# imazen/image-webp

Hardware: AMD Instinct MI355X
Metric: 1920x1080 lossy encodes/s (Q75, method 4) (higher is better)
Workload: dtype int32; 1 GPU; encode_frame_lossy 1920x1080 RGBA Q75 m4; device_batch=1024, distinct_frames=4, mbs_per_frame=8160, parallelism=frames sharded over 1 GPU(s), steps_pipelined=True, pipeline_lanes=2

## Files before the change

image-webp_amd/csrc/zw_enc_kernels.hip:

```cpp
#include "zw_dev.h"

#include <type_traits>

#include "zw_enc_rows.h"
#include "zw_enc_pairfinal.h"

#define ZW_PH_N 28

#ifdef ZW_NW
#define ZW_NW1 ZW_NW
#define ZW_NW2 ZW_NW
#endif
#ifndef ZW_NW1
#define ZW_NW1 12
#endif
#ifndef ZW_NW2
#define ZW_NW2 12
#endif
#define NW_MAX (ZW_NW1 > ZW_NW2 ? ZW_NW1 : ZW_NW2)
#ifndef ZW_DYN_PRIO
#define ZW_DYN_PRIO 1
#endif
#ifndef ZW_DYN_PRIO1
#define ZW_DYN_PRIO1 2
#endif
#ifndef ZW_P1_LUMA_MAX
#define ZW_P1_LUMA_MAX 3
#endif
#ifndef ZW_CHAIN_PRIO
#define ZW_CHAIN_PRIO 3
#endif
#ifndef ZW_LUMA_PRIO
#define ZW_LUMA_PRIO 0
#endif

template <int PASS> struct PassShape {
    static constexpr int NW = PASS == 1 ? ZW_NW1 : ZW_NW2;
    static constexpr int WG = NW * 64;
};

struct EncArgs {
    const uint8_t *Y, *U, *V;
    const uint8_t* alpha;
    const ZwFrameParams* params;
    const ZwLevelCosts* lcost;
    int8_t* derr;
    ZwMbOut* out;
    uint8_t *ry, *ru, *rv;
    size_t ysz, csz;
    int mbw, mbh, pass;
    int* dbg;
    uint8_t* rows;
    uint32_t* sizes;
    int nframes;
};

struct MbLds {
    uint8_t sy[256], su[64], sv[64];
    uint8_t ws[17 * ZW_BPS];
    uint8_t left_y[20], left_u[12], left_v[12], left_c[12];
    int8_t left_derr[4];
    uint8_t modes[16];
    int16_t lev[25][16];
};

struct WaveLds {
    MbLds mb;
    uint8_t cu[9 * ZW_BPS], cv[9 * ZW_BPS];
    uint32_t uvc[64][8];
    int dc[64];
    int y2d[64];
    int y2cost[4];
    int V[2][40];
    int nzt[4], nzl[4];
    int misc[16];
    uint32_t pst[2][4];
    uint8_t win_y[32], win_u[8], win_v[8], win_c[12];
    int8_t win_d[4];
#ifdef ZW_PHASE_PROF
    unsigned long long ph[ZW_PH_N];
#endif
};


struct Ctx {
    const EncArgs* a;
    const ZwFrameParams* P;
    int method;
    const ZwSegment* S;
    const ZwSegment* Sl;
    const LdsTables* T;
    WaveLds* W;
    MbLds* M;
    uint8_t *top_y, *top_u, *top_v, *top_c;
    int8_t* top_derr;
    const uint8_t *srcY, *srcU, *srcV;
    const uint8_t *sY, *sU, *sV;
    int ys, cs;
    int mbx, mby, lane, seg;
    int f;
    int oy, oc, ocx, od;
};

__device__ void build_luma_border(const Ctx& C, int part = 2)
{
    uint8_t* ws = C.M->ws;
    const int l = C.lane;
    const int mbw = C.a->mbw;
    const bool want = part == 2 || (part == 0 ? (l < 17 || l >= 32) : (l >= 17 && l < 32));
    if (!want) {
    } else if (l < 32) {
        int v;
        if (l == 0) v = C.mby == 0 ? 127 : (C.mbx == 0 ? 129 : C.M->left_y[0]);
        else if (C.mby == 0) v = 127;
        else if (l <= 16) v = C.top_y[C.oy + l - 1];
        else if (C.mbx == mbw - 1) v = C.top_y[C.oy + 15];
        else v = C.top_y[C.oy + l - 1];
        ws[l] = (uint8_t)v;
        if (l >= 17 && l < 21) {
            ws[4 * ZW_BPS + l] = (uint8_t)v;
            ws[8 * ZW_BPS + l] = (uint8_t)v;
            ws[12 * ZW_BPS + l] = (uint8_t)v;
        }
    } else if (l < 48) {
        int i = l - 32;
        ws[(i + 1) * ZW_BPS] = C.mbx == 0 ? 129 : C.M->left_y[1 + i];
    }
    wsync();
}

__device__ void build_chroma_border(const Ctx& C)
{
    const int l = C.lane;
    if (l < 34) {
        const int pl = l >= 17;
        const int i = pl ? l - 17 : l;
        uint8_t* w = pl ? C.W->cv : C.W->cu;
        const uint8_t* top = pl ? C.top_v : C.top_u;
        const uint8_t* left = pl ? C.M->left_v : C.M->left_u;
        if (i == 0) w[0] = C.mby == 0 ? 127 : (C.mbx == 0 ? 129 : left[0]);
        else if (i <= 8) w[i] = C.mby == 0 ? 127 : top[C.oc + i - 1];
        else w[(i - 8) * ZW_BPS] = C.mbx == 0 ? 129 : left[i - 8];
    }
    wsync();
}

template <int PASS>
__device__ void pick_i16(const Ctx& C, int& best_mode, unsigned long long& best_score)
{
    const int lane = C.lane, m = lane >> 4, b = lane & 15, bx = b & 3, by = b >> 2;
    const uint8_t* ws = C.M->ws;
    const ZwSegment& S = *C.S;
    const LdsTables* T = C.T;
    const int above = C.mby != 0, left = C.mbx != 0;
    int dcv;
    {
        const int top = lane < 16;
        const int v = (int)ws[csel(top, 1 + b, (b + 1) * ZW_BPS)] & -(int)(lane < 32 && (top ? above : left));
        const int sum = red16(v);
        const int s = __builtin_amdgcn_readlane(sum, 0) + __builtin_amdgcn_readlane(sum, 16);
        const int shf = 3 + above + left;
        dcv = (!above && !left) ? 128 : ((s + (1 << (shf - 1))) >> shf);
    }
    int src[16], pr[16], r[16], c[16];
    {
        const int P0 = ws[0];
        int L[4], Tp[4];
#pragma unroll
        for (int i = 0; i < 4; i++) {
            L[i] = ws[(by * 4 + i + 1) * ZW_BPS];
            Tp[i] = ws[1 + bx * 4 + i];
        }
#pragma unroll
        for (int i = 0; i < 4; i++) {
            const uint32_t srow = *(const uint32_t*)(C.sY + (by * 4 + i) * 16 + bx * 4);
#pragma unroll
            for (int j = 0; j < 4; j++) {
                const int p = sel4(m, dcv, Tp[j], L[i], clamp255(L[i] + Tp[j] - P0));
                const int sv = (int)((srow >> (8 * j)) & 255u);
                src[i * 4 + j] = sv;
                pr[i * 4 + j] = p;
                r[i * 4 + j] = sv - p;
            }
        }
    }
    fdct16_pk(r, c);
    int aq[16], dq[16];
    aq[0] = 0;
    int nzac = 0;
#pragma unroll
    for (int k = 1; k < 16; k++) {
        aq[k] = (int)((__umul24((uint32_t)iabs(c[k]), S.y1.iq[1]) + S.y1.bias[1]) >> 17);
        nzac |= aq[k];
        dq[k] = m24(c[k] < 0 ? -aq[k] : aq[k], (int)S.y1.q[1]);
    }
    nzac = nzac != 0;
    int cost = (int)rcost_bf<1, PASS == 2>(aq, 0, 0, T);
    int y2cost;
    {
        const int d = wht_g(c[0], b);
        const int t = b > 0;
        const int ay = (int)((__umul24((uint32_t)iabs(d), S.y2.iq[t]) + S.y2.bias[t]) >> 17);
        const int qy = d < 0 ? -ay : ay;
        y2cost = (int)rcost_g<0, PASS == 2>(qy, b, 0, 1, T);
        dq[0] = iwht_g(m24(qy, (int)S.y2.q[t]), b);
    }
    idct16(dq);
    int rec[16], sse = 0, flat = 1;
    const int s00 = C.sY[0];
#pragma unroll
    for (int k = 0; k < 16; k++) {
        rec[k] = clamp255(pr[k] + dq[k]);
        const int d = src[k] - rec[k];
        sse += m24(d, d);
        flat &= src[k] == s00;
    }
    int td = iabs(ttransform_diff_pk(rec, src)) >> 5;
    sse = red16(sse);
    td = red16(td);
    cost = red16(cost);
    nzac = red16(nzac);
    flat = red16(flat);
    const int srcflat = __builtin_amdgcn_readlane(flat, 0) == 16;
    cost += y2cost;
    int sd = S.tlambda > 0 ? ((int)S.tlambda * td + 128) >> 8 : 0;
    int dfin = sse;
    if (srcflat && nzac == 0) {
        dfin = sse * 2;
        sd = sd * 2;
    }
    const int mcost = sel4(m, d_FIXED_COSTS_I16[0], d_FIXED_COSTS_I16[1], d_FIXED_COSTS_I16[2], d_FIXED_COSTS_I16[3]) + cost;
    const int dist = dfin + sd;
    long long brd = 0x7fffffffffffffffLL, bfin = 0;
    int bm = 0;
#pragma unroll
    for (int mm = 0; mm < 4; mm++) {
        const long long mc = __builtin_amdgcn_readlane(mcost, mm * 16);
        const long long dd = 256LL * __builtin_amdgcn_readlane(dist, mm * 16);
        const long long r_m = mc * (long long)S.l_i16 + dd;
        const long long f_m = mc * (long long)S.l_mode + dd;
        const int avail = mm == 0 || (mm == 1 && above) || (mm == 2 && left) || (mm == 3 && above && left);
        if (avail && r_m < brd) {
            brd = r_m;
            bfin = f_m;
            bm = mm;
        }
    }
    best_mode = bm;
    best_score = bfin < 0 ? 0ull : (unsigned long long)bfin;
}

#ifdef ZW_PHASE_PROF
__device__ unsigned long long zw_phase_cycles_dev[2][ZW_PH_N];
__device__ unsigned long long zw_wave_cycles_dev[2][16][ZW_PH_N];
#define PH_START() long long ph_t_ = clock64()
#define PH_RESET() (ph_t_ = clock64())
#define PH_MARK(k) PH_MARK_L(k, lane, PASS)
#define PH_MARK_L(k, ln, ps)                                                        \
    do {                                                                            \
        const long long n_ = clock64();                                             \
        if ((ln) == 0) C.W->ph[k] += (unsigned long long)(n_ - ph_t_);               \
        ph_t_ = n_;                                                                 \
    } while (0)
extern "C" int zw_wave_cycles(unsigned long long* out, int reset)
{
    if (hipMemcpyFromSymbol(out, HIP_SYMBOL(zw_wave_cycles_dev), sizeof(zw_wave_cycles_dev)) != hipSuccess) return -1;
    if (reset) {
        static unsigned long long z[2][16][ZW_PH_N];
        if (hipMemcpyToSymbol(HIP_SYMBOL(zw_wave_cycles_dev), z, sizeof z) != hipSuccess) return -1;
    }
    return 0;
}
extern "C" int zw_phase_cycles(unsigned long long* out, int reset)
{
    if (hipMemcpyFromSymbol(out, HIP_SYMBOL(zw_phase_cycles_dev), sizeof(zw_phase_cycles_dev)) != hipSuccess) return -1;
    if (reset) {
        static unsigned long long z[2][ZW_PH_N];
        if (hipMemcpyToSymbol(HIP_SYMBOL(zw_phase_cycles_dev), z, sizeof z) != hipSuccess) return -1;
    }
    return 0;
}
#define PH_COUNT(k) \
    do {                \
        if (C.lane == 0) C.W->ph[k] += 1; \
    } while (0)
#else
#define PH_COUNT(k) (void)0
#define PH_START() (void)0
#define PH_RESET() (void)0
#define PH_MARK(k) (void)0
#define PH_MARK_L(k, ln, ps) (void)0
#endif

template <int NB>
__device__ __forceinline__ void i4_values_n(const Ctx& C, const int* x0, const int* y0)
{
    WaveLds* W = C.W;
    const uint8_t* ws = C.M->ws;
    const int l = C.lane;
    const int t = (int)(l >= 13) + (int)(l >= 24) + (int)(l >= 36) + (int)(l >= 37);
    const int k = min(l - 13 * (int)(l >= 13) - 11 * (int)(l >= 24), 12);
    const int t3 = (int)(t == 3), t4 = (int)(t >= 4), t12 = (int)(t == 1 || t == 2);
    const int ka = k + t3 * (11 - k) + t4 * (1 - k);
    const int kb = k + t12 + t3 * (12 - k) - t4 * k;
    const int kc = min(k + 2 * (int)(t == 1), 12);
    const int wb = 2 * (int)(t == 1) + (int)(t == 2) + 3 * (t3 + t4);
    const int wc = (int)(t == 1);
    const int sh = (int)(t != 0) + (int)(t != 0 && t != 2);
// ... 490 lines not shown
    const uint32_t rate = (uint32_t)(mcost + cost);
    const uint32_t score = (uint32_t)sse * 256u + (rate & 0xffffu) * S.l_i4;
    const uint32_t key2 = k < K ? (score << 2) | (uint32_t)k : 0xffffffffu;
    const uint32_t kmin = min16u(key2);
    const unsigned long long win = __ballot(key2 == kmin);
    PH_MARK_L(12, l, 0);
    int bk[NB];
#pragma unroll
    for (int h = 0; h < NB; h++) {
        bk[h] = __builtin_ctz((uint32_t)(win >> (16 * h)) & 0xffffu) >> 2;
        const int bmode = (int)((modes >> (16 * h + 4 * bk[h])) & 15u);
        const int wl = 16 * h + 4 * bk[h];
        const uint32_t bsse = (uint32_t)__builtin_amdgcn_readlane(sse, wl);
        const uint32_t brate = (uint32_t)__builtin_amdgcn_readlane((int)rate, wl);
        const int bnz = __builtin_amdgcn_readlane((int)(last >= 0), wl);
        const int i = sby[h] * 4 + sbx[h];
        st.tnz = (st.tnz & ~(1u << sbx[h])) | ((uint32_t)bnz << sbx[h]);
        st.lnz = (st.lnz & ~(1u << sby[h])) | ((uint32_t)bnz << sby[h]);
        st.nzm |= (uint32_t)bnz << i;
        st.total_mc += (uint32_t)__builtin_amdgcn_readlane(mcost, wl);
        st.running += rdscore(bsse, brate, S.l_mode);
        st.mpack |= (unsigned long long)bmode << (4 * i);
        if (l == h) C.M->modes[i] = (uint8_t)bmode;
    }
    const int bks = csel(slot, bk[sl], bk[0]);
    if (k == bks && l < 16 * NB) {
        const int xo = csel(slot, x0[sl], x0[0]), yo = csel(slot, y0[sl], y0[0]);
        const uint32_t wd = __builtin_amdgcn_perm(r32, r01, 0x04060200u);
        uint8_t* p = C.M->ws + (yo + q) * ZW_BPS + xo;
#pragma unroll
        for (int j = 0; j < 4; j++) p[j] = (uint8_t)(wd >> (8 * j));
        if (keep) {
            int16_t* lvp = C.M->lev[by * 4 + bx];
#pragma unroll
            for (int r = 0; r < 4; r++) lvp[izz_of(4 * r + q)] = (int16_t)lv[r];
        }
    }
    wsync();
    PH_MARK_L(13, l, 0);
}

template <int PASS, int NB>
__device__ __forceinline__ void i4_step(const Ctx& C, const int* sbx, const int* sby, int K, const I4Lane& LC,
                                        I4State& st, bool keep)
{
    const ZwSegment& S = *C.S;
    const LdsTables* T = C.T;
    const int l = C.lane, hf = l >> 5, m = l & 15;
    const int slot = NB == 2 ? (l >> 4) & 1 : 0;
    int x0[NB], y0[NB], tctx[NB], lctx[NB], nzc[NB];
#pragma unroll
    for (int h = 0; h < NB; h++) {
        const int i = sby[h] * 4 + sbx[h];
        x0[h] = sbx[h] * 4 + 1;
        y0[h] = sby[h] * 4 + 1;
        tctx[h] = sby[h] == 0 ? 0 : (int)((st.mpack >> (4 * (i - 4))) & 15);
        lctx[h] = sbx[h] == 0 ? 0 : (int)((st.mpack >> (4 * (i - 1))) & 15);
        nzc[h] = (sby[h] == 0 ? 0 : (int)((st.tnz >> sbx[h]) & 1)) + (sbx[h] == 0 ? 0 : (int)((st.lnz >> sby[h]) & 1));
    }
    const int sl = NB == 2 ? 1 : 0;
    const int bx = csel(slot, sbx[sl], sbx[0]), by = csel(slot, sby[sl], sby[0]);
    const int ctx0 = csel(slot, nzc[sl], nzc[0]);
    const int mcost = T->fci4[csel(slot, tctx[sl], tctx[0])][csel(slot, lctx[sl], lctx[0])][m < 10 ? m : 0];
    PH_START();
    const uint32_t vp = i4_values_pk<NB>(C, x0, y0);
    PH_MARK_L(10, l, 0);
    uint32_t ap01, ap32;
    {
        const uint32_t P = (uint32_t)__builtin_amdgcn_readlane((int)vp, 4);
        uint32_t a[4];
#pragma unroll
        for (int j = 0; j < 4; j++) a[j] = (uint32_t)__builtin_amdgcn_readlane((int)vp, 5 + j);
        const int sh = 16 * slot;
        const int p_ = (int)((P >> sh) & 255u);
        const int d0 = (int)((a[0] >> sh) & 255u) - p_, d1 = (int)((a[1] >> sh) & 255u) - p_;
        const int d2 = (int)((a[2] >> sh) & 255u) - p_, d3 = (int)((a[3] >> sh) & 255u) - p_;
        ap01 = pack_lo(d0, d1);
        ap32 = pack_lo(d3, d2);
    }
    uint32_t p01[2], p32[2];
#pragma unroll
    for (int r = 0; r < 2; r++) {
        const uint32_t ix = r ? LC.ib : LC.ia;
        const uint32_t v0 = (uint32_t)__builtin_amdgcn_ds_bpermute((int)(ix & 255u), (int)vp);
        const uint32_t v1 = (uint32_t)__builtin_amdgcn_ds_bpermute((int)((ix >> 8) & 255u), (int)vp);
        const uint32_t v2 = (uint32_t)__builtin_amdgcn_ds_bpermute((int)((ix >> 16) & 255u), (int)vp);
        const uint32_t v3 = (uint32_t)__builtin_amdgcn_ds_bpermute((int)(ix >> 24), (int)vp);
        const uint32_t q01 = __builtin_amdgcn_perm(v1, v0, LC.psel), q32 = __builtin_amdgcn_perm(v2, v3, LC.psel);
        p01[r] = LC.tm ? clamp_pk(add_pk(q01, ap01)) : q01;
        p32[r] = LC.tm ? clamp_pk(add_pk(q32, ap32)) : q32;
    }
    uint32_t s01[2], s32[2];
#pragma unroll
    for (int r = 0; r < 2; r++) {
        const uint32_t sw = *(const uint32_t*)(C.sY + (by * 4 + 2 * hf + r) * 16 + bx * 4);
        s01[r] = __builtin_amdgcn_perm(0u, sw, 0x0c010c00u);
        s32[r] = __builtin_amdgcn_perm(0u, sw, 0x0c020c03u);
    }
    int pse = 0;
#pragma unroll
    for (int r = 0; r < 2; r++) {
        const uint32_t d01 = sub_pk(s01[r], p01[r]), d32 = sub_pk(s32[r], p32[r]);
        pse = dot2v(d01, d01, pse);
        pse = dot2v(d32, d32, pse);
    }
    pse = hx_sum(pse);
    const int key = m < 10 ? (pse << 4) | m : 0x7fffffff;
    const int rank = rank16(key);
    PH_MARK_L(11, l, 0);
    if (K <= 4) {
        i4_cand_quad<PASS, NB>(C, sbx, sby, x0, y0, tctx, lctx, nzc, K, rank, vp, ap01, ap32, st, keep);
        return;
    }
    int cf[2][4];
    fdct_pair(s01, s32, p01, p32, hf, cf);
    int av[2][4], dq[2][4];
    unsigned sgn = 0;
    {
        const uint32_t iq0 = hf ? S.y1.iq[1] : S.y1.iq[0], bs0 = hf ? S.y1.bias[1] : S.y1.bias[0];
        const int q0 = hf ? (int)S.y1.q[1] : (int)S.y1.q[0];
#pragma unroll
        for (int c = 0; c < 2; c++)
#pragma unroll
            for (int r = 0; r < 4; r++) {
                const bool dcs = c == 0 && r == 0;
                const int v = cf[c][r];
                const int a = (int)((__umul24((uint32_t)iabs(v), dcs ? iq0 : S.y1.iq[1]) + (dcs ? bs0 : S.y1.bias[1])) >> 17);
                av[c][r] = a;
                dq[c][r] = m24(v < 0 ? -a : a, dcs ? q0 : (int)S.y1.q[1]);
                sgn |= (unsigned)(v < 0) << (4 * c + r);
            }
    }
    int last;
    const int cost = rcost_pair<PASS == 2>(av, hf, ctx0, 3, T, last);
    uint32_t r01[2], r32[2];
    idct_recon_pair(dq, p01, p32, hf, r01, r32);
    int sse = 0;
#pragma unroll
    for (int r = 0; r < 2; r++) {
        const uint32_t d01 = sub_pk(s01[r], r01[r]), d32 = sub_pk(s32[r], r32[r]);
        sse = dot2v(d01, d01, sse);
        sse = dot2v(d32, d32, sse);
    }
    sse = hx_sum(sse);
    const uint32_t rate = (uint32_t)(mcost + cost);
    const uint32_t score = (uint32_t)sse * 256u + (rate & 0xffffu) * S.l_i4;
    const bool elig = m < 10 && rank < K;
    const uint32_t sk = elig ? score : 0xffffffffu;
    const uint32_t smin = min16u(sk);
    const uint32_t rk = sk == smin ? (uint32_t)rank : 0xffffffffu;
    const uint32_t rmin = min16u(rk);
    const unsigned long long win = __ballot(rk == rmin && sk == smin);
    PH_MARK_L(12, l, 0);
    int bmode[NB];
#pragma unroll
    for (int h = 0; h < NB; h++) {
        bmode[h] = __builtin_ctz((uint32_t)(win >> (16 * h)) & 0xffffu);
        const int wl = 16 * h + bmode[h];
        const uint32_t bsse = (uint32_t)__builtin_amdgcn_readlane(sse, wl);
        const uint32_t brate = (uint32_t)__builtin_amdgcn_readlane((int)rate, wl);
        const int bnz = __builtin_amdgcn_readlane((int)(last >= 0), wl);
        const int i = sby[h] * 4 + sbx[h];
        st.tnz = (st.tnz & ~(1u << sbx[h])) | ((uint32_t)bnz << sbx[h]);
        st.lnz = (st.lnz & ~(1u << sby[h])) | ((uint32_t)bnz << sby[h]);
        st.nzm |= (uint32_t)bnz << i;
        st.total_mc += (uint32_t)__builtin_amdgcn_readlane(mcost, wl);
        st.running += rdscore(bsse, brate, S.l_mode);
        st.mpack |= (unsigned long long)bmode[h] << (4 * i);
        if (l == h) C.M->modes[i] = (uint8_t)bmode[h];
    }
    const int bms = csel(slot, bmode[sl], bmode[0]);
    if (m == bms && (NB == 2 || slot == 0)) {
        const int xo = csel(slot, x0[sl], x0[0]), yo = csel(slot, y0[sl], y0[0]);
#pragma unroll
        for (int r = 0; r < 2; r++) {
            const uint32_t wd = __builtin_amdgcn_perm(r32[r], r01[r], 0x04060200u);
            uint8_t* p = C.M->ws + (yo + 2 * hf + r) * ZW_BPS + xo;
#pragma unroll
            for (int j = 0; j < 4; j++) p[j] = (uint8_t)(wd >> (8 * j));
        }
        if (keep) {
            int16_t* lv = C.M->lev[by * 4 + bx];
#pragma unroll
            for (int c = 0; c < 2; c++)
#pragma unroll
                for (int r = 0; r < 4; r++) {
                    const int a = av[c][r];
                    lv[izz_of(4 * r + 2 * hf + c)] = (int16_t)(((sgn >> (4 * c + r)) & 1u) ? -a : a);
                }
        }
    }
    wsync();
    PH_MARK_L(13, l, 0);
}

template <int PASS>
__device__ bool pick_i4(const Ctx& C, unsigned long long i16_score, bool keep, uint32_t& nzm)
{
    const ZwSegment& S = *C.S;
    const int K = C.method <= 3 ? 3 : (C.method == 4 ? 4 : 10);
    I4State st;
    st.running = 211ull * S.l_mode;
    st.total_mc = 0;
    st.mpack = 0;
    st.tnz = st.lnz = st.nzm = 0;
    I4Lane LC;
    i4_lane_init(C, LC);
    PH_COUNT(20);
    for (int s = 0; s < 10; s++) {
        PH_COUNT(19);
        const int sbyA = s < 4 ? 0 : (s - 2) >> 1;
        const int sbxA = s - 2 * sbyA;
        if (s >= 2 && s <= 7) {
            const int bx[2] = {sbxA, sbxA - 2}, by[2] = {sbyA, sbyA + 1};
            i4_step<PASS, 2>(C, bx, by, K, LC, st, keep);
        } else {
            i4_step<PASS, 1>(C, &sbxA, &sbyA, K, LC, st, keep);
        }
        if (st.running >= i16_score) return false;
        if (st.total_mc > 256u * 16u * 16u / 4u) return false;
    }
    nzm = st.nzm;
    return true;
}

struct I4PLane {
    uint32_t ix[4];
    uint32_t psel;
    int tm;
    uint32_t iq0, bs0, iq1, bs1;
    int q0, qa;
    uint32_t l_i4;
};

DI uint32_t i4p_psel(int hm, int slot)
{
    const uint32_t b = (uint32_t)(2 * hm + slot);
    return 0x0c000c00u | ((4u + b) << 16) | b;
}

DI void i4p_lane_init(const Ctx& C, const Ctx& CB, I4PLane& L)
{
    const int l = C.lane, m = l & 15, mv = m < 10 ? m : 0;
    {
        const ZwSegment* Sh = (l >> 5) ? CB.S : C.S;
        const int q = l & 3;
        L.iq0 = q ? Sh->y1.iq[1] : Sh->y1.iq[0];
        L.bs0 = q ? Sh->y1.bias[1] : Sh->y1.bias[0];
        L.iq1 = Sh->y1.iq[1];
        L.bs1 = Sh->y1.bias[1];
        L.q0 = q ? (int)Sh->y1.q[1] : (int)Sh->y1.q[0];
        L.qa = (int)Sh->y1.q[1];
        L.l_i4 = Sh->l_i4;
    }
#pragma unroll
    for (int r = 0; r < 4; r++) {
        uint32_t w = 0;
#pragma unroll
        for (int j = 0; j < 4; j++) w |= (uint32_t)(4 * (i4_src_index(C.T, mv, 4 * r + j) & 255)) << (8 * j);
        L.ix[r] = w;
    }
    L.psel = i4p_psel(l >> 5, (l >> 4) & 1);
    L.tm = mv == 1;
}

template <int NB>
DI uint32_t i4p_values(const Ctx& CA, const Ctx& CB, const int* x0, const int* y0)
{
    const int l = CA.lane;
    const int t = (int)(l >= 13) + (int)(l >= 24) + (int)(l >= 36) + (int)(l >= 37);
    const int k = min(l - 13 * (int)(l >= 13) - 11 * (int)(l >= 24), 12);
    const int t3 = (int)(t == 3), t4 = (int)(t >= 4), t12 = (int)(t == 1 || t == 2);
    const int ka = k + t3 * (11 - k) + t4 * (1 - k);
    const int kb = k + t12 + t3 * (12 - k) - t4 * k;
    const int kc = min(k + 2 * (int)(t == 1), 12);
    const int wb = 2 * (int)(t == 1) + (int)(t == 2) + 3 * (t3 + t4);
    const int wc = (int)(t == 1);
    const int sh = (int)(t != 0) + (int)(t != 0 && t != 2);
    const int oa = csel(ka < 4, -ka * ZW_BPS, ka - 4 - 4 * ZW_BPS);
    const int ob = csel(kb < 4, -kb * ZW_BPS, kb - 4 - 4 * ZW_BPS);
    const int oc = csel(kc < 4, -kc * ZW_BPS, kc - 4 - 4 * ZW_BPS);
    const bool dcl = l < 4 || (l >= 5 && l < 9);
    uint32_t v[2], ea[2];
#pragma unroll
    for (int mb = 0; mb < 2; mb++) {
        const uint8_t* ws = (mb ? CB : CA).M->ws;
        v[mb] = ea[mb] = 0;
#pragma unroll
        for (int h = 0; h < 2; h++) {
            const int hh = NB == 2 ? h : 0;
            const int rowL = (y0[hh] + 3) * ZW_BPS + x0[hh] - 1;
            const int a = ws[rowL + oa], eb = ws[rowL + ob], ec = ws[rowL + oc];
            v[mb] |= (uint32_t)((a + wb * eb + wc * ec + ((1 << sh) >> 1)) >> sh) << (16 * h);
            ea[mb] |= (uint32_t)a << (16 * h);
        }
    }
    const uint32_t da = (uint32_t)__builtin_amdgcn_readfirstlane(red16((int)(dcl ? ea[0] : 0u)));
    const uint32_t db = (uint32_t)__builtin_amdgcn_readfirstlane(red16((int)(dcl ? ea[1] : 0u)));
    const uint32_t dcv = (((da & 0xffffu) + 4) >> 3) | ((((da >> 16) + 4) >> 3) << 8) |
                         ((((db & 0xffffu) + 4) >> 3) << 16) | ((((db >> 16) + 4) >> 3) << 24);
    return l == 38 ? dcv : __builtin_amdgcn_perm(v[1], v[0], 0x06040200u);
}

template <int PASS, int NB>
DI void i4p_step(const Ctx& CA, const Ctx& CB, const int* sbx, const int* sby, int K, const I4PLane& LC,
                 I4State st[2], const bool act[2], bool keep)
{
    [[maybe_unused]] const Ctx& C = CA;
    const int l = CA.lane, m = l & 15, hm = l >> 5;
    const int slot = NB == 2 ? (l >> 4) & 1 : 0;
    const int sl = NB == 2 ? 1 : 0;
    int x0[NB], y0[NB], tc[2][NB], lc[2][NB], nc[2][NB];
#pragma unroll
    for (int h = 0; h < NB; h++) {
        const int i = sby[h] * 4 + sbx[h];
        x0[h] = sbx[h] * 4 + 1;
        y0[h] = sby[h] * 4 + 1;
#pragma unroll
        for (int mb = 0; mb < 2; mb++) {
            tc[mb][h] = sby[h] == 0 ? 0 : (int)((st[mb].mpack >> (4 * (i - 4))) & 15);
            lc[mb][h] = sbx[h] == 0 ? 0 : (int)((st[mb].mpack >> (4 * (i - 1))) & 15);
            nc[mb][h] = (sby[h] == 0 ? 0 : (int)((st[mb].tnz >> sbx[h]) & 1)) +
                        (sbx[h] == 0 ? 0 : (int)((st[mb].lnz >> sby[h]) & 1));
        }
    }
    auto pick = [&](const int (&v)[2][NB]) {
        const int a = csel(slot, v[0][sl], v[0][0]), b = csel(slot, v[1][sl], v[1][0]);
        return csel(hm, b, a);
    };
    const int tctx = pick(tc), lctx = pick(lc), ctx0 = pick(nc);
    const int bx = csel(slot, sbx[sl], sbx[0]), by = csel(slot, sby[sl], sby[0]);
    const uint8_t* sYh = hm ? CB.sY : CA.sY;
    const LdsTables* Th = hm ? CB.T : CA.T;
    PH_START();
    const uint32_t vp = i4p_values<NB>(CA, CB, x0, y0);
    uint32_t ap01, ap32;
    {
        const uint32_t P = (uint32_t)__builtin_amdgcn_readlane((int)vp, 4);
        uint32_t a[4];
#pragma unroll
        for (int j = 0; j < 4; j++) a[j] = (uint32_t)__builtin_amdgcn_readlane((int)vp, 5 + j);
        const int sh = 8 * (2 * hm + slot);
        const int p_ = (int)((P >> sh) & 255u);
        const int d0 = (int)((a[0] >> sh) & 255u) - p_, d1 = (int)((a[1] >> sh) & 255u) - p_;
        const int d2 = (int)((a[2] >> sh) & 255u) - p_, d3 = (int)((a[3] >> sh) & 255u) - p_;
        ap01 = pack_lo(d0, d1);
        ap32 = pack_lo(d3, d2);
    }
    PH_MARK_L(10, l, 0);
    int pse = 0;
#pragma unroll
    for (int r = 0; r < 4; r++) {
        const uint32_t ix = LC.ix[r];
        const uint32_t v0 = (uint32_t)__builtin_amdgcn_ds_bpermute((int)(ix & 255u), (int)vp);
        const uint32_t v1 = (uint32_t)__builtin_amdgcn_ds_bpermute((int)((ix >> 8) & 255u), (int)vp);
        const uint32_t v2 = (uint32_t)__builtin_amdgcn_ds_bpermute((int)((ix >> 16) & 255u), (int)vp);
        const uint32_t v3 = (uint32_t)__builtin_amdgcn_ds_bpermute((int)(ix >> 24), (int)vp);
        const uint32_t q01 = __builtin_amdgcn_perm(v1, v0, LC.psel), q32 = __builtin_amdgcn_perm(v2, v3, LC.psel);
        const uint32_t p01 = LC.tm ? clamp_pk(add_pk(q01, ap01)) : q01;
        const uint32_t p32 = LC.tm ? clamp_pk(add_pk(q32, ap32)) : q32;
        const uint32_t sw = *(const uint32_t*)(sYh + (by * 4 + r) * 16 + bx * 4);
        const uint32_t d01 = sub_pk(__builtin_amdgcn_perm(0u, sw, 0x0c010c00u), p01);
        const uint32_t d32 = sub_pk(__builtin_amdgcn_perm(0u, sw, 0x0c020c03u), p32);
        pse = dot2v(d01, d01, pse);
        pse = dot2v(d32, d32, pse);
    }
    const int key = m < 10 ? (pse << 4) | m : 0x7fffffff;
    const int rank = rank16(key);
    PH_MARK_L(11, l, 0);
    unsigned long long modes = 0;
    for (int k = 0; k < K; k++) {
        const unsigned long long b = __ballot(m < 10 && rank == k);
#pragma unroll
        for (int g = 0; g < 4; g++)
            modes |= (unsigned long long)__builtin_ctz((uint32_t)(b >> (16 * g)) | 0x10000u) << (16 * g + 4 * k);
    }
    const int k = (l >> 2) & 3, q = l & 3;
    const int g = 2 * hm + slot;
    const int mq = (int)((modes >> (16 * g + 4 * k)) & 15ull);
    const int mv = k < K ? mq : 0;
    const int mcost = Th->fci4[tctx][lctx][mv];
    const uint32_t iq0 = LC.iq0, bs0 = LC.bs0, iq1 = LC.iq1, bs1 = LC.bs1;
    const int q0 = LC.q0, qa = LC.qa;
    int hn[2];
    hn[0] = (int)Th->binit[3][0][ctx0] & -(int)(ctx0 == 0);
    hn[1] = (int)Th->beob[3][0][ctx0];
    uint32_t p01, p32;
    {
        const uint32_t iw = *(const uint32_t*)&Th->i4qa[mv][4 * q];
        uint32_t v[4];
#pragma unroll
        for (int j = 0; j < 4; j++)
            v[j] = (uint32_t)__builtin_amdgcn_ds_bpermute((int)((iw >> (8 * j)) & 255u), (int)vp);
        const uint32_t q01 = __builtin_amdgcn_perm(v[1], v[0], LC.psel), q32 = __builtin_amdgcn_perm(v[2], v[3], LC.psel);
        const bool tm = mv == 1;
        p01 = tm ? clamp_pk(add_pk(q01, ap01)) : q01;
        p32 = tm ? clamp_pk(add_pk(q32, ap32)) : q32;
    }
    uint32_t s01, s32;
    {
        const uint32_t sw = *(const uint32_t*)(sYh + (by * 4 + q) * 16 + bx * 4);
        s01 = __builtin_amdgcn_perm(0u, sw, 0x0c010c00u);
        s32 = __builtin_amdgcn_perm(0u, sw, 0x0c020c03u);
    }
    PH_MARK_L(22, l, 0);
    const uint32_t R01 = sub_pk(s01, p01), R32 = sub_pk(s32, p32);
    int cf[4];
    uvq_fdct(add_pk(R01, R32), sub_pk(R01, R32), q, cf);
    int av[4], dq[4], lv[4];
#pragma unroll
    for (int r = 0; r < 4; r++) {
        const bool dcs = r == 0;
        const int v = cf[r];
        const int a = (int)((__umul24((uint32_t)iabs(v), dcs ? iq0 : iq1) + (dcs ? bs0 : bs1)) >> 17);
        av[r] = a;
        lv[r] = v < 0 ? -a : a;
        dq[r] = m24(lv[r], dcs ? q0 : qa);
    }
    int last;
    const int cost = rcost_quad<PASS == 2>(av, q, ctx0, 3, Th, last, hn);
    PH_MARK_L(23, l, 0);
    uint32_t r01, r32;
    uvq_idct_recon(dq, p01, p32, q, r01, r32);
    int sse = 0;
    {
        const uint32_t d01 = sub_pk(s01, r01), d32 = sub_pk(s32, r32);
        sse = dot2v(d01, d01, sse);
        sse = dot2v(d32, d32, sse);
    }
    sse = quad_sum(sse);
    const uint32_t rate = (uint32_t)(mcost + cost);
    const uint32_t score = (uint32_t)sse * 256u + (rate & 0xffffu) * LC.l_i4;
    const uint32_t key2 = k < K ? (score << 2) | (uint32_t)k : 0xffffffffu;
    const uint32_t kmin = min16u(key2);
    const unsigned long long win = __ballot(key2 == kmin);
    const uint32_t pk = (rate & 0xffffu) | ((uint32_t)mcost << 16) | ((uint32_t)(last >= 0) << 31);
    PH_MARK_L(12, l, 0);
#pragma unroll
    for (int mb = 0; mb < 2; mb++) {
        const ZwSegment& S = *(mb ? CB : CA).S;
        MbLds* M = (mb ? CB : CA).M;
#pragma unroll
        for (int h = 0; h < NB; h++) {
            const int gg = 2 * mb + h;
            const int bk = __builtin_ctz((uint32_t)(win >> (16 * gg)) & 0xffffu) >> 2;
            const int bmode = (int)((modes >> (16 * gg + 4 * bk)) & 15ull);
            const int wl = 16 * gg + 4 * bk;
            const uint32_t bsse = (uint32_t)__builtin_amdgcn_readlane(sse, wl);
            const uint32_t bpk = (uint32_t)__builtin_amdgcn_readlane((int)pk, wl);
            const uint32_t brate = bpk & 0xffffu;
            const int bnz = (int)(bpk >> 31);
            const int i = sby[h] * 4 + sbx[h];
            I4State& s = st[mb];
            s.tnz = (s.tnz & ~(1u << sbx[h])) | ((uint32_t)bnz << sbx[h]);
            s.lnz = (s.lnz & ~(1u << sby[h])) | ((uint32_t)bnz << sby[h]);
            s.nzm |= (uint32_t)bnz << i;
            s.total_mc += (bpk >> 16) & 0x7fffu;
            s.running += rdscore(bsse, brate, S.l_mode);
            s.mpack |= (unsigned long long)bmode << (4 * i);
            if (act[mb] && l == gg) M->modes[i] = (uint8_t)bmode;
        }
    }
    const int bks = __builtin_ctz((uint32_t)(win >> (16 * g)) & 0xffffu) >> 2;
    if (k == bks && ((l >> 4) & 1) < NB && (hm ? act[1] : act[0])) {
        MbLds* M = hm ? CB.M : CA.M;
        const int xo = csel(slot, x0[sl], x0[0]), yo = csel(slot, y0[sl], y0[0]);
        const uint32_t wd = __builtin_amdgcn_perm(r32, r01, 0x04060200u);
        uint8_t* p = M->ws + (yo + q) * ZW_BPS + xo;
#pragma unroll
        for (int j = 0; j < 4; j++) p[j] = (uint8_t)(wd >> (8 * j));
        if (keep) {
            int16_t* lvp = M->lev[by * 4 + bx];
#pragma unroll
            for (int r = 0; r < 4; r++) lvp[izz_of(4 * r + q)] = (int16_t)lv[r];
        }
    }
    wsync();
    PH_MARK_L(13, l, 0);
}

template <int PASS>
__device__ uint32_t pick_i4_pair(const Ctx& CA, const Ctx& CB, unsigned long long i16A, unsigned long long i16B,
                                 bool actA, bool actB, bool keep, uint32_t& nzA, uint32_t& nzB)
{
    const int K = CA.method <= 3 ? 3 : 4;
    I4State st[2];
    st[0].running = 211ull * CA.S->l_mode;
    st[1].running = 211ull * CB.S->l_mode;
#pragma unroll
    for (int mb = 0; mb < 2; mb++) {
        st[mb].total_mc = 0;
        st[mb].mpack = 0;
        st[mb].tnz = st[mb].lnz = st[mb].nzm = 0;
    }
    bool act[2] = {actA, actB};
    const unsigned long long lim[2] = {i16A, i16B};
    I4PLane LC;
    i4p_lane_init(CA, CB, LC);
    for (int s = 0; s < 10; s++) {
        const int sbyA = s < 4 ? 0 : (s - 2) >> 1;
        const int sbxA = s - 2 * sbyA;
        if (s >= 2 && s <= 7) {
            const int bx[2] = {sbxA, sbxA - 2}, by[2] = {sbyA, sbyA + 1};
            i4p_step<PASS, 2>(CA, CB, bx, by, K, LC, st, act, keep);
        } else {
            i4p_step<PASS, 1>(CA, CB, &sbxA, &sbyA, K, LC, st, act, keep);
        }
#pragma unroll
        for (int mb = 0; mb < 2; mb++)
            if (st[mb].running >= lim[mb] || st[mb].total_mc > 256u * 16u * 16u / 4u) act[mb] = false;
        if (!act[0] && !act[1]) return 0;
    }
    nzA = st[0].nzm;
    nzB = st[1].nzm;
    return (uint32_t)act[0] | ((uint32_t)act[1] << 1);
}

__device__ int final_luma(const Ctx& C, int mode, bool trel, int y_nz_out[16], int i4_nzm)
{
    WaveLds* W = C.W;
    const ZwSegment& S = *C.S;
    const int l = C.lane;
    int anynz = 0;
    PH_START();
    if (mode == 4 && i4_nzm >= 0) {
#pragma unroll
        for (int i = 0; i < 16; i++) y_nz_out[i] = (i4_nzm >> i) & 1;
        if (l < 16) C.M->lev[16][l] = 0;
        wsync();
        PH_MARK_L(15, l, 0);
        PH_COUNT(7);
        return i4_nzm != 0;
    }
    if (mode != 4) {
        build_luma_border(C);
        const uint8_t* ws = C.M->ws;
        const int above = C.mby != 0, left = C.mbx != 0;
        const int b = l & 15, bx = b & 3, by = b >> 2;
        int dcv;
        {
            const int top = l < 16;
            const int v = (int)ws[csel(top, 1 + b, (b + 1) * ZW_BPS)] & -(int)(l < 32 && (top ? above : left));
            const int sum = red16(v);
            const int su = __builtin_amdgcn_readlane(sum, 0) + __builtin_amdgcn_readlane(sum, 16);
            const int shf = 3 + above + left;
            dcv = (!above && !left) ? 128 : ((su + (1 << (shf - 1))) >> shf);
        }
        int c[16], pr[16];
        {
            const int P0 = ws[0];
            int L[4], Tp[4], r[16];
#pragma unroll
            for (int i = 0; i < 4; i++) {
                L[i] = ws[(by * 4 + i + 1) * ZW_BPS];
                Tp[i] = ws[1 + bx * 4 + i];
            }
#pragma unroll
            for (int i = 0; i < 4; i++) {
                const uint32_t srow = *(const uint32_t*)(C.sY + (by * 4 + i) * 16 + bx * 4);
#pragma unroll
                for (int j = 0; j < 4; j++) {
                    const int p = sel4(mode, dcv, Tp[j], L[i], clamp255(L[i] + Tp[j] - P0));
                    pr[i * 4 + j] = p;
                    r[i * 4 + j] = (int)((srow >> (8 * j)) & 255u) - p;
                }
            }
            fdct16_pk(r, c);
        }
        int y2dq;
        {
            const int d = wht_g(c[0], b);
            const int t = b > 0;
            const int y2q = quantz(d, S.y2.iq[t], S.y2.bias[t]);
            if (l < 16) C.M->lev[16][izz_of(b)] = (int16_t)y2q;
            if (gmask(y2q != 0)) anynz = 1;
            y2dq = iwht_g(m24(y2q, (int)S.y2.q[t]), b);
        }
        PH_MARK_L(16, l, 0);
        int dq[16], lv[16];
        int nzb = 0;
        {
            int snz = 0;
            if (l < 16) {
#pragma unroll
                for (int k = 1; k < 16; k++) snz |= quantz(c[k], S.y1.iq[1], S.y1.bias[1]) != 0;
            }
            anynz |= __any(snz) ? 1 : 0;
        }
        if (trel) {
            int tnz = 0;
            if (l < 48) {
#pragma unroll
                for (int k = 0; k < 16; k++) dq[k] = c[k];
                tnz = trellis<1, true>(dq, lv, S.y1, S.sharpen, S.lt_i16, C.T, 0, l >> 4);
            }
            PH_MARK_L(17, l, 0);
            const unsigned long long nzm = __ballot(l < 48 && tnz);
            int nt[4], nl[4];
#pragma unroll
            for (int q = 0; q < 4; q++) {
                nt[q] = __builtin_amdgcn_readfirstlane(C.top_c[C.ocx + 1 + q]);
                nl[q] = __builtin_amdgcn_readfirstlane(C.M->left_c[1 + q]);
            }
            unsigned code = 0, nzbits = 0;
#pragma unroll
            for (int bb = 0; bb < 16; bb++) {
                const int cx = min(nl[bb >> 2] + nt[bb & 3], 2);
                const int z = (int)((nzm >> (cx * 16 + bb)) & 1ull);
                nt[bb & 3] = z;
                nl[bb >> 2] = z;
                code |= (unsigned)cx << (2 * bb);
                nzbits |= (unsigned)z << bb;
            }
            const int srcl = (int)((code >> (2 * b)) & 3u) * 16 + b;
            lv[0] = 0;
#pragma unroll
            for (int i = 0; i < 8; i++) {
                const uint32_t w = (uint32_t)__shfl((int)pack_lo(lv[2 * i], lv[2 * i + 1]), srcl);
                lv[2 * i] = lo16(w);
                lv[2 * i + 1] = hi16(w);
            }
#pragma unroll
            for (int n = 1; n < 16; n++) dq[kZZ(n)] = m24(lv[n], (int)S.y1.q[1]);
            nzb = (nzbits >> b) & 1u;
            PH_MARK_L(18, l, 0);
        } else if (l < 16) {
#pragma unroll
            for (int n = 1; n < 16; n++) {
                const int j = kZZ(n);
                lv[n] = quantz(c[j], S.y1.iq[1], S.y1.bias[1]);
                nzb |= lv[n] != 0;
            }
            dq[0] = 0;
#pragma unroll
            for (int n = 1; n < 16; n++) dq[kZZ(n)] = m24(lv[n], (int)S.y1.q[1]);
        }
        wsync();
        if (l < 16) {
            lv[0] = 0;
#pragma unroll
            for (int n = 0; n < 16; n++) C.M->lev[b][n] = (int16_t)lv[n];
            dq[0] = y2dq;
            idct16(dq);
            uint8_t* wsp = C.M->ws;
#pragma unroll
            for (int k = 0; k < 16; k++) {
                const int y = by * 4 + (k >> 2), x = bx * 4 + (k & 3);
                wsp[(y + 1) * ZW_BPS + 1 + x] = (uint8_t)clamp255(pr[k] + dq[k]);
            }
        }
        const unsigned nzmask = (unsigned)__ballot(l < 16 && nzb);
        for (int k = 0; k < 16; k++) y_nz_out[k] = (int)((nzmask >> k) & 1u);
        wsync();
        PH_MARK_L(14, l, 0);
    } else {
        build_luma_border(C);
        int top_nz[4], left_nz[4];
        for (int k = 0; k < 4; k++) {
            top_nz[k] = C.top_c[C.ocx + 1 + k];
            left_nz[k] = C.M->left_c[1 + k];
        }
        for (int i = 0; i < 16; i++) {
            const int sby = i >> 2, sbx = i & 3, x0 = sbx * 4 + 1, y0 = sby * 4 + 1;
            const int bm = C.M->modes[i];
            i4_values(C, x0, y0);
            const int k = l & 15;
            const int pk = i4_pred_at(W->V[0], i4_src_index(C.T, bm, k), W->V[0][5 + (k & 3)] - W->V[0][4]);
            const int svk = C.sY[(sby * 4 + (k >> 2)) * 16 + sbx * 4 + (k & 3)];
            const int ck = fdct_g(svk - pk, k);
            const int ctx0 = min(left_nz[sby] + top_nz[sbx], 2);
            if (C.a->dbg && C.a->pass == 2 && l < 16) {
                int* d = C.a->dbg + (((size_t)C.f * C.a->mbw * C.a->mbh + (size_t)C.mby * C.a->mbw + C.mbx) * 16 + i) * 34;
                d[k] = ck;
                d[16 + k] = pk;
                if (k == 0) {
                    d[32] = ctx0;
                    d[33] = bm;
                }
            }
            const int qs = quantz(ck, S.y1.iq[k > 0], S.y1.bias[k > 0]);
            const int snz = gmask(qs != 0) != 0;
            int dqk, nzq;
            if (trel) {
                const int cn = gget(ck, zz_of(k));
                int lvn;
                nzq = trellis_g<0>(cn, k, S.y1, S.sharpen, S.lt_i4, C.T, 3, ctx0, lvn);
                if (l < 16) C.M->lev[i][k] = (int16_t)lvn;
                dqk = m24(gget(lvn, izz_of(k)), (int)S.y1.q[k > 0]);
            } else {
                if (l < 16) C.M->lev[i][izz_of(k)] = (int16_t)qs;
                nzq = snz;
                dqk = m24(qs, (int)S.y1.q[k > 0]);
            }
            const int rk = idct_g(dqk, k);
            if (l < 16) C.M->ws[(y0 + (k >> 2)) * ZW_BPS + x0 + (k & 3)] = (uint8_t)clamp255(pk + rk);
            wsync();
            if (l == 0) {
                W->misc[1] = nzq;
                W->misc[2] = snz;
            }
            wsync();
            const int nz = W->misc[1];
            anynz |= W->misc[2];
            top_nz[sbx] = nz;
            left_nz[sby] = nz;
            y_nz_out[i] = nz;
            wsync();
        }
        if (l < 16) C.M->lev[16][l] = 0;
        wsync();
        PH_MARK_L(15, l, 0);
        PH_COUNT(7);
    }
    return anynz;
}

__device__ void final_luma_pair(const Ctx& CA, const Ctx& CB, int modeA, int modeB, bool trel, uint32_t& resA,
                                uint32_t& resB)
{
    [[maybe_unused]] const Ctx& C = CA;
    WaveLds* W = CA.W;
    const int l = CA.lane, hm = l >> 5, b = l & 15, bx = b & 3, by = b >> 2;
    const bool own = (l & 16) == 0;
    PH_START();
    build_luma_border(CA);
    build_luma_border(CB);
    MbLds* const M = hm ? CB.M : CA.M;
    const ZwSegment* const S = hm ? CB.S : CA.S;
    const uint8_t* const sY = hm ? CB.sY : CA.sY;
    const int mode = hm ? modeB : modeA;
    const uint8_t* ws = M->ws;
    const int above = CA.mby != 0, left = CA.mbx != 0;
    int dcv;
    {
        const int v = (int)ws[csel(own, 1 + b, (b + 1) * ZW_BPS)] & -(int)(own ? above : left);
        const int sum = red16(v);
        const int sa = __builtin_amdgcn_readlane(sum, 0) + __builtin_amdgcn_readlane(sum, 16);
        const int sb = __builtin_amdgcn_readlane(sum, 32) + __builtin_amdgcn_readlane(sum, 48);
        const int shf = 3 + above + left;
        dcv = (!above && !left) ? 128 : (((hm ? sb : sa) + (1 << (shf - 1))) >> shf);
    }
    int c[16];
    uint32_t ppk[4];
    {
        const int P0 = ws[0];
        int L[4], Tp[4], r[16];
#pragma unroll
        for (int i = 0; i < 4; i++) {
            L[i] = ws[(by * 4 + i + 1) * ZW_BPS];
            Tp[i] = ws[1 + bx * 4 + i];
        }
#pragma unroll
        for (int i = 0; i < 4; i++) {
            const uint32_t srow = *(const uint32_t*)(sY + (by * 4 + i) * 16 + bx * 4);
            ppk[i] = 0;
#pragma unroll
            for (int j = 0; j < 4; j++) {
                const int p = sel4(mode, dcv, Tp[j], L[i], clamp255(L[i] + Tp[j] - P0));
                ppk[i] |= (uint32_t)p << (8 * j);
                r[i * 4 + j] = (int)((srow >> (8 * j)) & 255u) - p;
            }
        }
        fdct16_pk(r, c);
    }
    int y2dq;
    uint32_t anyA, anyB;
    {
        const int d = wht_g(c[0], b);
        const int t = b > 0;
        const int y2q = quantz(d, S->y2.iq[t], S->y2.bias[t]);
        if (own) M->lev[16][izz_of(b)] = (int16_t)y2q;
        y2dq = iwht_g(m24(y2q, (int)S->y2.q[t]), b);
        int snz = y2q != 0;
        const uint32_t iq1 = S->y1.iq[1], bs1 = S->y1.bias[1];
#pragma unroll
        for (int k = 1; k < 16; k++) snz |= quantz(c[k], iq1, bs1) != 0;
        const unsigned long long any = __ballot(snz != 0);
        anyA = (uint32_t)any != 0u;
        anyB = (uint32_t)(any >> 32) != 0u;
    }
    PH_MARK_L(16, l, 0);
    const int q1 = (int)S->y1.q[1];
    int nzb = 0;
    auto finish = [&](bool act, int* lv) {
        wsync();
        if (act) {
            int dq[16];
            lv[0] = 0;
#pragma unroll
            for (int n = 0; n < 16; n++) M->lev[b][n] = (int16_t)lv[n];
#pragma unroll
            for (int n = 1; n < 16; n++) dq[kZZ(n)] = m24(lv[n], q1);
            dq[0] = y2dq;
            idct16(dq);
            uint8_t* wsp = M->ws;
#pragma unroll
            for (int k = 0; k < 16; k++) {
                const int y = by * 4 + (k >> 2), x = bx * 4 + (k & 3);
                const int p = (int)((ppk[k >> 2] >> (8 * (k & 3))) & 255u);
                wsp[(y + 1) * ZW_BPS + 1 + x] = (uint8_t)clamp255(p + dq[k]);
            }
        }
    };
    if (trel) {
        const bool tzl = pf_trivial(c, (uint32_t)q1, S->y1.iq[1], S->sharpen);
        const unsigned long long tzb = __ballot(tzl);
        const unsigned tzA = (unsigned)tzb & 0xffffu, tzB = (unsigned)(tzb >> 32) & 0xffffu;
        unsigned eA = 0, eB = 0;
#pragma unroll
        for (int q = 0; q < 4; q++) {
            eA |= (unsigned)(__builtin_amdgcn_readfirstlane(CA.top_c[CA.ocx + 1 + q]) != 0) << q;
            eA |= (unsigned)(__builtin_amdgcn_readfirstlane(CA.M->left_c[1 + q]) != 0) << (4 + q);
            eB |= (unsigned)(__builtin_amdgcn_readfirstlane(CB.top_c[CB.ocx + 1 + q]) != 0) << q;
            eB |= (unsigned)(__builtin_amdgcn_readfirstlane(CB.M->left_c[1 + q]) != 0) << (4 + q);
        }
        unsigned long long mA = 0, mB = 0;
        {
// ... 1471 lines not shown
```

Before: 4630 encodes/s.

## Keep I4 pair search state per lane and invert mode ranking via ds_permute

Replaces the wave-uniform per-macroblock I4 state, which needed a ballot and readlane for every winner, with compact per-lane state. Winners are broadcast with row rotations and permlane16_swap, and contexts are read directly from packed lane state. The top-K mode selection now uses a single ds_permute that inverts the rank instead of a ballot loop over K. Context-dependent LDS reads are hoisted earlier so they overlap the prediction SSE pass. This cuts scalar readlane and ballot serialization in the hot 4x4 intra search, at the cost of more VGPR state and relying on permlane16_swap, a newer instruction.

```diff
diff --git a/image-webp_amd/csrc/zw_enc_i4pair.h b/image-webp_amd/csrc/zw_enc_i4pair.h
--- /dev/null
+++ b/image-webp_amd/csrc/zw_enc_i4pair.h
@@ -0,0 +1,83 @@
+#pragma once
+#include <stdint.h>
+
+#ifndef ZW_HD
+#ifdef __HIPCC__
+#define ZW_HD __host__ __device__
+#else
+#define ZW_HD
+#endif
+#endif
+
+#ifndef ZW_I4P_INV
+#define ZW_I4P_INV 1
+#endif
+#ifndef ZW_I4P_LANES
+#define ZW_I4P_LANES 1
+#endif
+
+#define ZW_I4P_KMAX 4
+
+ZW_HD inline int i4p_inv_dest(int lane, int rank)
+{
+    return (lane & ~15) + (rank < ZW_I4P_KMAX ? 4 * rank : 1);
+}
+ZW_HD inline int i4p_mode_src(int lane) { return lane & ~3; }
+ZW_HD inline bool i4p_eligible(int lane, int K) { return ((lane >> 2) & 3) < K; }
+ZW_HD inline int i4p_mode(int lane, int K, int received) { return i4p_eligible(lane, K) ? received : 0; }
+
+struct I4PWin {
+    uint32_t pk;
+    uint32_t sm;
+};
+ZW_HD inline I4PWin i4p_win(uint32_t rate, uint32_t mcost, bool nz, uint32_t sse, int mode)
+{
+    I4PWin w;
+    w.pk = (rate & 0xffffu) | (mcost << 16) | ((uint32_t)nz << 31);
+    w.sm = sse | ((uint32_t)mode << 24);
+    return w;
+}
+
+struct I4PState {
+    uint64_t running;
+    uint32_t total_mc;
+    uint32_t nzt;
+    uint32_t lm;
+};
+
+ZW_HD inline void i4p_state_init(I4PState& s, uint32_t l_mode)
+{
+    s.running = 211ull * l_mode;
+    s.total_mc = 0;
+    s.nzt = 0;
+    s.lm = 0;
+}
+
+ZW_HD inline void i4p_state_update(I4PState& s, int bx, int by, I4PWin w, uint32_t l_mode)
+{
+    const uint32_t mode = w.sm >> 24, sse = w.sm & 0xffffffu;
+    s.nzt |= (w.pk >> 31) << (by * 4 + bx);
+    s.nzt = (s.nzt & ~(0xf0000u << (4 * bx))) | (mode << (16 + 4 * bx));
+    s.lm = (s.lm & ~(0xfu << (4 * by))) | (mode << (4 * by));
+    s.total_mc += (w.pk >> 16) & 0x7fffu;
+    s.running += (uint64_t)sse * 256ull + (uint64_t)(w.pk & 0xffffu) * l_mode;
+}
+
+ZW_HD inline int i4p_tctx(const I4PState& s, int bx, int by)
+{
+    return by == 0 ? 0 : (int)((s.nzt >> (16 + 4 * bx)) & 15u);
+}
+ZW_HD inline int i4p_lctx(const I4PState& s, int bx, int by)
+{
+    return bx == 0 ? 0 : (int)((s.lm >> (4 * by)) & 15u);
+}
+ZW_HD inline int i4p_nzctx(const I4PState& s, int bx, int by)
+{
+    const int i = by * 4 + bx;
+    return (by == 0 ? 0 : (int)((s.nzt >> ((i - 4) & 15)) & 1u)) + (bx == 0 ? 0 : (int)((s.nzt >> ((i - 1) & 15)) & 1u));
+}
+
+ZW_HD inline bool i4p_exit(const I4PState& s, uint64_t i16_score)
+{
+    return s.running >= i16_score || s.total_mc > 256u * 16u * 16u / 4u;
+}
diff --git a/image-webp_amd/csrc/zw_enc_kernels.hip b/image-webp_amd/csrc/zw_enc_kernels.hip
--- a/image-webp_amd/csrc/zw_enc_kernels.hip
+++ b/image-webp_amd/csrc/zw_enc_kernels.hip
@@ -4,6 +4,7 @@
 
 #include "zw_enc_rows.h"
 #include "zw_enc_pairfinal.h"
+#include "zw_enc_i4pair.h"
 
 #define ZW_PH_N 28
 
@@ -1100,26 +1101,42 @@
     return l == 38 ? dcv : __builtin_amdgcn_perm(v[1], v[0], 0x06040200u);
 }
 
+#if ZW_I4P_LANES
+typedef I4PState I4PSearch;
+#else
+struct I4PSearch {
+    I4State mb[2];
+};
+#endif
+
 template <int PASS, int NB>
 DI void i4p_step(const Ctx& CA, const Ctx& CB, const int* sbx, const int* sby, int K, const I4PLane& LC,
-                 I4State st[2], const bool act[2], bool keep)
+                 I4PSearch& st, const bool act[2], bool keep)
 {
     [[maybe_unused]] const Ctx& C = CA;
     const int l = CA.lane, m = l & 15, hm = l >> 5;
     const int slot = NB == 2 ? (l >> 4) & 1 : 0;
     const int sl = NB == 2 ? 1 : 0;
-    int x0[NB], y0[NB], tc[2][NB], lc[2][NB], nc[2][NB];
+    int x0[NB], y0[NB];
+#pragma unroll
+    for (int h = 0; h < NB; h++) {
+        x0[h] = sbx[h] * 4 + 1;
+        y0[h] = sby[h] * 4 + 1;
+    }
+    const int bx = csel(slot, sbx[sl], sbx[0]), by = csel(slot, sby[sl], sby[0]);
+#if ZW_I4P_LANES
+    const int tctx = i4p_tctx(st, bx, by), lctx = i4p_lctx(st, bx, by), ctx0 = i4p_nzctx(st, bx, by);
+#else
+    int tc[2][NB], lc[2][NB], nc[2][NB];
 #pragma unroll
     for (int h = 0; h < NB; h++) {
         const int i = sby[h] * 4 + sbx[h];
-        x0[h] = sbx[h] * 4 + 1;
-        y0[h] = sby[h] * 4 + 1;
 #pragma unroll
         for (int mb = 0; mb < 2; mb++) {
-            tc[mb][h] = sby[h] == 0 ? 0 : (int)((st[mb].mpack >> (4 * (i - 4))) & 15);
-            lc[mb][h] = sbx[h] == 0 ? 0 : (int)((st[mb].mpack >> (4 * (i - 1))) & 15);
-            nc[mb][h] = (sby[h] == 0 ? 0 : (int)((st[mb].tnz >> sbx[h]) & 1)) +
-                        (sbx[h] == 0 ? 0 : (int)((st[mb].lnz >> sby[h]) & 1));
+            tc[mb][h] = sby[h] == 0 ? 0 : (int)((st.mb[mb].mpack >> (4 * (i - 4))) & 15);
+            lc[mb][h] = sbx[h] == 0 ? 0 : (int)((st.mb[mb].mpack >> (4 * (i - 1))) & 15);
+            nc[mb][h] = (sby[h] == 0 ? 0 : (int)((st.mb[mb].tnz >> sbx[h]) & 1)) +
+                        (sbx[h] == 0 ? 0 : (int)((st.mb[mb].lnz >> sby[h]) & 1));
         }
     }
     auto pick = [&](const int (&v)[2][NB]) {
@@ -1127,9 +1144,19 @@
         return csel(hm, b, a);
     };
     const int tctx = pick(tc), lctx = pick(lc), ctx0 = pick(nc);
-    const int bx = csel(slot, sbx[sl], sbx[0]), by = csel(slot, sby[sl], sby[0]);
+#endif
     const uint8_t* sYh = hm ? CB.sY : CA.sY;
     const LdsTables* Th = hm ? CB.T : CA.T;
+    const int k = (l >> 2) & 3, q = l & 3;
+    int hn[2];
+    uint32_t swq;
+    const uint16_t* fcrow;
+    auto read_ctx = [&]() {
+        hn[0] = (int)Th->binit[3][0][ctx0] & -(int)(ctx0 == 0);
+        hn[1] = (int)Th->beob[3][0][ctx0];
+        swq = *(const uint32_t*)(sYh + (by * 4 + q) * 16 + bx * 4);
+        fcrow = Th->fci4[tctx][lctx];
+    };
     PH_START();
     const uint32_t vp = i4p_values<NB>(CA, CB, x0, y0);
     uint32_t ap01, ap32;
@@ -1146,6 +1173,9 @@
         ap32 = pack_lo(d3, d2);
     }
     PH_MARK_L(10, l, 0);
+#if ZW_I4P_INV
+    read_ctx();
+#endif
     int pse = 0;
 #pragma unroll
     for (int r = 0; r < 4; r++) {
@@ -1166,23 +1196,23 @@
     const int key = m < 10 ? (pse << 4) | m : 0x7fffffff;
     const int rank = rank16(key);
     PH_MARK_L(11, l, 0);
+#if ZW_I4P_INV
+    const int mv = i4p_mode(l, K, qb0(__builtin_amdgcn_ds_permute(4 * i4p_inv_dest(l, rank), m)));
+#else
     unsigned long long modes = 0;
-    for (int k = 0; k < K; k++) {
-        const unsigned long long b = __ballot(m < 10 && rank == k);
+    for (int kk = 0; kk < K; kk++) {
+        const unsigned long long b = __ballot(m < 10 && rank == kk);
 #pragma unroll
         for (int g = 0; g < 4; g++)
-            modes |= (unsigned long long)__builtin_ctz((uint32_t)(b >> (16 * g)) | 0x10000u) << (16 * g + 4 * k);
-    }
-    const int k = (l >> 2) & 3, q = l & 3;
-    const int g = 2 * hm + slot;
-    const int mq = (int)((modes >> (16 * g + 4 * k)) & 15ull);
+            modes |= (unsigned long long)__builtin_ctz((uint32_t)(b >> (16 * g)) | 0x10000u) << (16 * g + 4 * kk);
+    }
+    const int mq = (int)((modes >> (16 * (2 * hm + slot) + 4 * k)) & 15ull);
     const int mv = k < K ? mq : 0;
-    const int mcost = Th->fci4[tctx][lctx][mv];
+    read_ctx();
+#endif
+    const int mcost = fcrow[mv];
     const uint32_t iq0 = LC.iq0, bs0 = LC.bs0, iq1 = LC.iq1, bs1 = LC.bs1;
     const int q0 = LC.q0, qa = LC.qa;
-    int hn[2];
-    hn[0] = (int)Th->binit[3][0][ctx0] & -(int)(ctx0 == 0);
-    hn[1] = (int)Th->beob[3][0][ctx0];
     uint32_t p01, p32;
     {
         const uint32_t iw = *(const uint32_t*)&Th->i4qa[mv][4 * q];
@@ -1195,12 +1225,8 @@
         p01 = tm ? clamp_pk(add_pk(q01, ap01)) : q01;
         p32 = tm ? clamp_pk(add_pk(q32, ap32)) : q32;
     }
-    uint32_t s01, s32;
-    {
-        const uint32_t sw = *(const uint32_t*)(sYh + (by * 4 + q) * 16 + bx * 4);
-        s01 = __builtin_amdgcn_perm(0u, sw, 0x0c010c00u);
-        s32 = __builtin_amdgcn_perm(0u, sw, 0x0c020c03u);
-    }
+    const uint32_t s01 = __builtin_amdgcn_perm(0u, swq, 0x0c010c00u);
+    const uint32_t s32 = __builtin_amdgcn_perm(0u, swq, 0x0c020c03u);
     PH_MARK_L(22, l, 0);
     const uint32_t R01 = sub_pk(s01, p01), R32 = sub_pk(s32, p32);
     int cf[4];
@@ -1231,6 +1257,37 @@
     const uint32_t score = (uint32_t)sse * 256u + (rate & 0xffffu) * LC.l_i4;
     const uint32_t key2 = k < K ? (score << 2) | (uint32_t)k : 0xffffffffu;
     const uint32_t kmin = min16u(key2);
+    const bool actl = hm ? act[1] : act[0];
+#if ZW_I4P_LANES
+    const bool winl = key2 == kmin && k < K;
+    PH_MARK_L(12, l, 0);
+    {
+        const I4PWin own = i4p_win(rate, (uint32_t)mcost, last >= 0, (uint32_t)sse, mv);
+        uint32_t w0 = winl ? own.pk : 0u, w1 = winl ? own.sm : 0u;
+        w0 |= (uint32_t)ror8((int)w0);
+        w1 |= (uint32_t)ror8((int)w1);
+        w0 |= (uint32_t)ror4((int)w0);
+        w1 |= (uint32_t)ror4((int)w1);
+        const uint32_t lml = hm ? CB.S->l_mode : CA.S->l_mode;
+        if (NB == 2) {
+            const auto p0 = __builtin_amdgcn_permlane16_swap(w0, w0, false, false);
+            const auto p1 = __builtin_amdgcn_permlane16_swap(w1, w1, false, false);
+#pragma unroll
+            for (int h = 0; h < 2; h++) {
+                I4PWin w;
+                w.pk = p0[h];
+                w.sm = p1[h];
+                i4p_state_update(st, sbx[h], sby[h], w, lml);
+            }
+        } else {
+            I4PWin w;
+            w.pk = w0;
+            w.sm = w1;
+            i4p_state_update(st, sbx[0], sby[0], w, lml);
+        }
+        if (actl && m == 0 && ((l >> 4) & 1) < NB) (hm ? CB.M : CA.M)->modes[by * 4 + bx] = (uint8_t)(w1 >> 24);
+    }
+#else
     const unsigned long long win = __ballot(key2 == kmin);
     const uint32_t pk = (rate & 0xffffu) | ((uint32_t)mcost << 16) | ((uint32_t)(last >= 0) << 31);
     PH_MARK_L(12, l, 0);
@@ -1242,14 +1299,18 @@
         for (int h = 0; h < NB; h++) {
             const int gg = 2 * mb + h;
             const int bk = __builtin_ctz((uint32_t)(win >> (16 * gg)) & 0xffffu) >> 2;
+            const int wl = 16 * gg + 4 * bk;
+#if ZW_I4P_INV
+            const int bmode = __builtin_amdgcn_readlane(mv, wl);
+#else
             const int bmode = (int)((modes >> (16 * gg + 4 * bk)) & 15ull);
-            const int wl = 16 * gg + 4 * bk;
+#endif
             const uint32_t bsse = (uint32_t)__builtin_amdgcn_readlane(sse, wl);
             const uint32_t bpk = (uint32_t)__builtin_amdgcn_readlane((int)pk, wl);
             const uint32_t brate = bpk & 0xffffu;
             const int bnz = (int)(bpk >> 31);
             const int i = sby[h] * 4 + sbx[h];
-            I4State& s = st[mb];
+            I4State& s = st.mb[mb];
             s.tnz = (s.tnz & ~(1u << sbx[h])) | ((uint32_t)bnz << sbx[h]);
             s.lnz = (s.lnz & ~(1u << sby[h])) | ((uint32_t)bnz << sby[h]);
             s.nzm |= (uint32_t)bnz << i;
@@ -1259,8 +1320,9 @@
             if (act[mb] && l == gg) M->modes[i] = (uint8_t)bmode;
         }
     }
-    const int bks = __builtin_ctz((uint32_t)(win >> (16 * g)) & 0xffffu) >> 2;
-    if (k == bks && ((l >> 4) & 1) < NB && (hm ? act[1] : act[0])) {
+    const bool winl = k == (__builtin_ctz((uint32_t)(win >> (16 * (2 * hm + slot))) & 0xffffu) >> 2);
+#endif
+    if (winl && ((l >> 4) & 1) < NB && actl) {
         MbLds* M = hm ? CB.M : CA.M;
         const int xo = csel(slot, x0[sl], x0[0]), yo = csel(slot, y0[sl], y0[0]);
         const uint32_t wd = __builtin_amdgcn_perm(r32, r01, 0x04060200u);
@@ -1282,17 +1344,21 @@
                                  bool actA, bool actB, bool keep, uint32_t& nzA, uint32_t& nzB)
 {
     const int K = CA.method <= 3 ? 3 : 4;
-    I4State st[2];
-    st[0].running = 211ull * CA.S->l_mode;
-    st[1].running = 211ull * CB.S->l_mode;
+    I4PSearch st;
+#if ZW_I4P_LANES
+    i4p_state_init(st, (CA.lane >> 5) ? CB.S->l_mode : CA.S->l_mode);
+#else
+    st.mb[0].running = 211ull * CA.S->l_mode;
+    st.mb[1].running = 211ull * CB.S->l_mode;
 #pragma unroll
     for (int mb = 0; mb < 2; mb++) {
-        st[mb].total_mc = 0;
-        st[mb].mpack = 0;
-        st[mb].tnz = st[mb].lnz = st[mb].nzm = 0;
-    }
+        st.mb[mb].total_mc = 0;
+        st.mb[mb].mpack = 0;
+        st.mb[mb].tnz = st.mb[mb].lnz = st.mb[mb].nzm = 0;
+    }
+    const unsigned long long lim[2] = {i16A, i16B};
+#endif
     bool act[2] = {actA, actB};
-    const unsigned long long lim[2] = {i16A, i16B};
     I4PLane LC;
     i4p_lane_init(CA, CB, LC);
     for (int s = 0; s < 10; s++) {
@@ -1304,13 +1370,23 @@
         } else {
             i4p_step<PASS, 1>(CA, CB, &sbxA, &sbyA, K, LC, st, act, keep);
         }
+#if ZW_I4P_LANES
+        if (__ballot(i4p_exit(st, i16A)) & 1ull) act[0] = false;
+        if ((__ballot(i4p_exit(st, i16B)) >> 32) & 1ull) act[1] = false;
+#else
 #pragma unroll
         for (int mb = 0; mb < 2; mb++)
-            if (st[mb].running >= lim[mb] || st[mb].total_mc > 256u * 16u * 16u / 4u) act[mb] = false;
+            if (st.mb[mb].running >= lim[mb] || st.mb[mb].total_mc > 256u * 16u * 16u / 4u) act[mb] = false;
+#endif
         if (!act[0] && !act[1]) return 0;
     }
-    nzA = st[0].nzm;
-    nzB = st[1].nzm;
+#if ZW_I4P_LANES
+    nzA = (uint32_t)__builtin_amdgcn_readlane((int)st.nzt, 0) & 0xffffu;
+    nzB = (uint32_t)__builtin_amdgcn_readlane((int)st.nzt, 32) & 0xffffu;
+#else
+    nzA = st.mb[0].nzm;
+    nzB = st.mb[1].nzm;
+#endif
     return (uint32_t)act[0] | ((uint32_t)act[1] << 1);
 }
 
```

Measured after the change: 4973 encodes/s (median of 6 runs). +7.4%, better.
